# rust-seq/simd-minimizers

Measured on AMD Instinct MI355X. Metric: Gbases/s (whole node) for canonical minimizers k=21 w=11 on 3.1 Gbp; HBM GB/s %peak, higher is better.
Workload: dtype u32

## Files before the change

include/simd_minimizers_amd.h:

```cpp
#ifndef SIMD_MINIMIZERS_AMD_H
#define SIMD_MINIMIZERS_AMD_H

#include <stddef.h>
#include <stdint.h>

#ifdef __cplusplus
extern "C" {
#endif


typedef struct mm_hasher {
    uint32_t fw[4];
    uint32_t rc[4];
    uint32_t rot;
    uint32_t canonical;
    uint32_t fw_xor;
    uint32_t rc_xor;
    uint32_t kind;
} mm_hasher_t;

typedef enum mm_hasher_kind { MM_HASHER_NT = 0, MM_HASHER_MUL = 1, MM_HASHER_ANTILEX = 2 } mm_hasher_kind_t;

typedef enum mm_mode { MM_MINIMIZERS = 0, MM_CLOSED_SYNCMERS = 1, MM_OPEN_SYNCMERS = 2 } mm_mode_t;

// ... 564 lines not shown
int mm_device_group_batch_result(const mm_device_group_t *group, uint64_t seq, int *entry, uint32_t **d_pos,
                                 uint32_t **d_sk, uint64_t *count);
int mm_device_group_gather_batch(mm_device_group_t *group, int root, uint32_t *d_dst_pos, uint32_t *d_dst_sk ,
                                 uint64_t capacity, uint64_t *out_offsets );
int mm_device_group_values_batch(mm_device_group_t *group, uint32_t len, int canonical, int want_u128, uint64_t *total);
int mm_device_group_batch_values(const mm_device_group_t *group, uint64_t seq, int *entry, uint64_t **d_values,
                                 uint64_t *count);

int mm_debug_launch_plan(uint32_t w, int canonical_windows, int mode, uint64_t n_seqs, const uint64_t *n_windows,
                         uint64_t *out7, uint32_t *tile_seq, uint32_t *tile_win0, uint32_t *tile_nblk,
                         uint64_t tile_capacity, uint64_t *n_tiles);
int mm_debug_launch_lds(uint32_t w, int canonical_windows, int mode, uint64_t n_windows, uint64_t *out2);
int mm_debug_fixed_k_kernel(uint32_t k, uint32_t w, int canonical_windows);
int mm_debug_kc_count(uint32_t w, uint32_t k, uint32_t kn, uint32_t jj, uint32_t group, const uint8_t *bytes,
                      uint64_t n_bytes, int64_t lane_base, uint32_t *count);
#define MM_TRAIT_WIDE_GROUP_BLOCKS 0
#define MM_TRAIT_WIDE_DWORDS 1
#define MM_TRAIT_V2_LOAD 2
#define MM_TRAIT_VIEW_WORDS 3
#define MM_TRAIT_AMB_VIEW_WORDS 4
#define MM_TRAIT_SK_SHIFT 5
#define MM_TRAIT_AMBI_LAND 6
#define MM_TRAIT_AMBI_ROWS 7
#define MM_TRAIT_AMB_ROW_DWORDS 8
#define MM_TRAIT_LAZY_VOTE 9
#define MM_TRAIT_TABLE_PREFETCH 10
#define MM_TRAIT_TWO_BODIES 11
#define MM_TRAIT_ENTRY8 12
#define MM_TRAIT_ONE_STREAM 13
#define MM_TRAIT_LAST_VIEW_BASES 14
// ... 17 lines not shown
```

simd-minimizers_amd/__init__.py:

```python
from __future__ import annotations

import ctypes as C
import os
import threading

import numpy as np

_HERE = os.path.dirname(os.path.abspath(__file__))
LIB_PATH = os.environ.get("MM_LIB_PATH") or os.path.join(_HERE, "libsimd_minimizers_amd.so")

MM_MINIMIZERS, MM_CLOSED_SYNCMERS, MM_OPEN_SYNCMERS = 0, 1, 2
PATH_FUSED, PATH_GENERIC, PATH_SPLIT = 1, 2, 3
U64_MAX = (1 << 64) - 1

ERR = {
    "W_ZERO": -1, "W_TOO_LARGE": -2, "LEN_TOO_LARGE": -3, "EVEN_L": -4,
    "HASHER_NOT_CANONICAL": -5, "OPEN_EVEN_W": -6, "K_ZERO": -7, "CAPACITY": -8, "BAD_MODE": -9,
    "NULL": -10, "VALUE_LEN": -11, "FORMAT": -12, "NO_DEVICE": -20, "HIP": -21, "ALLOC": -22, "ORDER": -23,
    "UNSORTED": -24,
}


class MinimizerError(RuntimeError):
    def __init__(self, code: int, msg: str):
# ... 133 lines not shown
                                                           C.c_uint32, vp, vp, C.c_uint64, vp, vp]
            L.mm_run_packed_reads_device.argtypes = [vp, vp, vp, C.c_uint64, C.c_uint64, C.c_uint64, vp, C.c_uint64,
                                                     C.c_uint32, vp, vp, C.c_uint64, vp, u64p]
            L.mm_run_packed_reads_host.argtypes = [vp, vp, u8p, C.c_uint64, u64p, C.c_uint32, u32p, u32p, C.c_uint64, u64p, u64p]
            L.mm_debug_launch_plan.argtypes = [C.c_uint32, C.c_int, C.c_int, C.c_uint64, u64p, u64p, u32p, u32p, u32p,
                                               C.c_uint64, u64p]
        L.mm_clock_probe_begin.argtypes = [vp, C.c_uint64]
        L.mm_clock_probe_end.argtypes = [vp, C.POINTER(C.c_double)]
        L.mm_link_probe.argtypes = [vp, vp, vp, C.c_uint64, C.POINTER(C.c_double)]
        L.mm_debug_launch_lds.argtypes = [C.c_uint32, C.c_int, C.c_int, C.c_uint64, u64p]
        L.mm_debug_fixed_k_kernel.argtypes = [C.c_uint32, C.c_uint32, C.c_int]
        if hasattr(L, "mm_debug_kc_count"):
            L.mm_debug_kc_count.argtypes = [C.c_uint32, C.c_uint32, C.c_uint32, C.c_uint32, C.c_uint32, u8p, C.c_uint64,
                                            C.c_int64, u32p]
            L.mm_debug_kc_count.restype = C.c_int
        if hasattr(L, "mm_debug_walk_traits"):
            L.mm_debug_walk_traits.argtypes = [C.c_uint32, C.c_int, C.c_int, C.c_int, C.c_int, C.c_int, u32p, C.c_int]
            L.mm_debug_walk_traits.restype = C.c_int
        L.mm_debug_lane_plan.argtypes = [C.c_uint32, C.c_uint32, C.c_int, C.c_int, C.c_uint64, C.c_uint64, C.c_uint32, u64p]
        L.mm_debug_last_lane_table.argtypes = [vp, u32p, C.c_uint64, u64p]
        L.mm_fused_overread_bytes.argtypes = []
        L.mm_fused_overread_bytes.restype = C.c_uint64
        L.mm_workspace_force_generic.argtypes = [vp, C.c_int]
        L.mm_workspace_set_blocks_per_lane.argtypes = [vp, C.c_uint32]
        L.mm_workspace_enable_timing.argtypes = [vp, C.c_int]
        L.mm_workspace_kernel_time.argtypes = [vp, C.POINTER(C.c_double), u64p, C.c_int]
        L.mm_workspace_last_path.argtypes = [vp]
        L.mm_workspace_ticket_mode.argtypes = [vp]
        L.mm_workspace_last_lane_table.argtypes = [vp]
        if hasattr(L, "mm_prebuilt_window_sizes"):
# ... 228 lines not shown
    "mm_debug_text_counts_view",
    "mm_run_packed_reads_counts_device_async", "mm_run_packed_reads_counts_device",
    "mm_run_packed_reads_skip_ambiguous_counts_device_async", "mm_run_packed_reads_skip_ambiguous_counts_device",
    "mm_debug_lane_counts_view",
    "mm_fastx_stream_create", "mm_fastx_stream_feed", "mm_fastx_stream_finish", "mm_fastx_stream_next",
    "mm_fastx_stream_destroy", "mm_debug_fastx_cut", "mm_fastx_stream_pieces", "mm_debug_fastx_split",
    "mm_one_minimizer_reads_device_async", "mm_one_minimizer_text_batch_device_async", "mm_one_minimizer_reads_host",
    "mm_one_minimizer_text_batch_host", "mm_one_minimizer_tile", "mm_debug_one_minimizer_reads",
    "mm_debug_one_minimizer_text_batch",
    "mm_one_minimizer_text_batch_counts_device_async", "mm_one_minimizer_reads_counts_device_async",
    "mm_debug_one_minimizer_counts_view", "mm_debug_one_minimizer_text_batch_counts", "mm_debug_one_minimizer_reads_counts",
    "mm_fastx_text_stream_create", "mm_fastx_text_stream_extras",
    "mm_one_minimizer_reads_skip_ambiguous_device_async", "mm_one_minimizer_reads_skip_ambiguous_counts_device_async",
    "mm_one_minimizer_reads_skip_ambiguous_host", "mm_debug_one_minimizer_reads_skip_ambiguous",
    "mm_debug_one_minimizer_reads_skip_ambiguous_counts", "mm_fastx_stream_one_minimizer",
    "mm_debug_walk_traits", "mm_debug_kc_count",
    "mm_bgzf_scan_host", "mm_bgzf_inflate_device_async", "mm_bgzf_inflate_host", "mm_debug_bgzf_inflate",
    "mm_fastx_stream_feed_bgzf",
]

WALK_TRAITS = ("wide_group_blocks", "wide_dwords", "v2_load", "view_words", "amb_view_words", "sk_shift", "ambi_land",
               "ambi_rows", "amb_row_dwords", "lazy_vote", "table_prefetch", "two_bodies", "entry8", "one_stream",
               "last_view_bases")


def walk_traits(w: int, canonical: bool, mode: int = 0, super_kmers: bool = False, reads: bool = False,
                ambiguous: bool = False) -> dict:
    L = lib()
    n = L.mm_debug_walk_traits(int(w), int(canonical), int(mode), int(super_kmers), int(reads), int(ambiguous), None, 0)
    if n != len(WALK_TRAITS):
        raise RuntimeError(f"mm_debug_walk_traits lists {n} values, this package knows {len(WALK_TRAITS)}")
# ... 2125 lines not shown
```

simd-minimizers_amd/csrc/mm_api.hip:

```cpp
#include <hip/hip_runtime.h>

#include <cstdio>
#include <cstdlib>
#include <chrono>
#include <cstring>
#include <new>
#include <algorithm>
#include <string>
#include <thread>
#include <utility>
#include <vector>

#include "../../include/simd_minimizers_amd.h"
#include "mm_env.h"
#include "mm_launch.h"
#include "mm_fasta_text.h"
#include "mm_lane_counts.h"
#include "mm_text_counts.h"
#include "mm_values_batch.h"
#include "mm_values_block.h"
#include "mm_one_min.h"
#include "mm_values_reads.h"
#include "mm_values_text.h"
#include "mm_bgzf.h"
// ... 960 lines not shown
    mm::fused_debug_lds(a, o);
    out2[0] = o[0];
    out2[1] = o[1];
    return MM_OK;
}

int mm_debug_fixed_k_kernel(uint32_t k, uint32_t w, int canonical_windows) {
    return mm::fused_fixed_k(k, w, canonical_windows, canonical_windows) ? 1 : 0;
}

int mm_debug_kc_count(uint32_t w, uint32_t k, uint32_t kn, uint32_t jj, uint32_t group, const uint8_t *bytes, uint64_t n_bytes,
                      int64_t lane_base, uint32_t *count) {
    return mm::fused_kc_count(w, k, kn, jj, group, bytes, n_bytes, lane_base, count);
}

static_assert(MM_WALK_TRAITS == mm::kWalkTraits, "the header's trait indices and fused_walk_traits list the same fields");
int mm_debug_walk_traits(uint32_t w, int canonical_windows, int mode, int super_kmers, int reads, int ambiguous, uint32_t *out,
                         int capacity) {
    if (w == 0 || mode < 0 || mode > 2) return 0;
    return mm::fused_walk_traits(w, canonical_windows != 0, (uint32_t)mode, super_kmers != 0, reads != 0, ambiguous != 0, out,
                                 capacity < 0 ? 0 : capacity);
}

int mm_debug_launch_plan(uint32_t w, int canonical_windows, int mode, uint64_t n_seqs, const uint64_t *n_windows,
                         uint64_t *out7, uint32_t *tile_seq, uint32_t *tile_win0, uint32_t *tile_nblk, uint64_t tile_capacity,
                         uint64_t *n_tiles) {
    ApiScope api_scope;
    if (!n_windows || w == 0) return MM_ERR_NULL;
    mm::RunArgs a = debug_plan_args(w, canonical_windows, mode, n_seqs, n_windows[0]);
    if (n_seqs == 0) {
// ... 4382 lines not shown
```

simd-minimizers_amd/csrc/mm_fused.hip:

```cpp
#include "mm_fused_impl.h"
#include "mm_fused_inst.h"
#include "mm_env.h"
#include "mm_launch.h"
#include "mm_split.h"

#include <cstdlib>
#include <cstdio>
#include <map>
#include <mutex>
#include <string>
#include <utility>
#include <vector>

namespace mm {

namespace {

using KernelFn = FusedKernelFn;
using Instance = FusedInstance;

uint32_t debug_switches() {
#ifdef MM_EXPERIMENTS
    const char *dbg = mm_exp_env("MM_DEBUG");
    return dbg ? (uint32_t)atoi(dbg) : 0u;
// ... 23 lines not shown
    }
    return nullptr;
}

const FusedKcInstance *find_kc_instance(uint32_t w, uint32_t k, int canonical_windows, int hasher_canonical) {
    if (mm_exp_env("MM_NO_KC")) return nullptr;
    int n = 0;
    const FusedKcInstance *inst = fused_kc_instances(&n);
    for (int i = 0; i < n; ++i)
        if (inst[i].w == w && inst[i].k == k && inst[i].canon == (canonical_windows != 0) &&
            inst[i].hash_rc == (hasher_canonical != 0))
            return &inst[i];
    return nullptr;
}

double emit_density(uint32_t w, uint32_t mode) {
    return mode == 2 ? 1.0 / w : (mode == 1 ? 2.0 / w : 2.0 / (w + 1.0));
}

uint32_t list_capacity(uint32_t w, uint32_t mode, uint32_t S) {
    static const uint32_t extra = mm_exp_env("MM_CAP_EXTRA") ? (uint32_t)atoi(mm_exp_env("MM_CAP_EXTRA")) : 0u;
    uint32_t cap = (uint32_t)(1.3 * emit_density(w, mode) * S) + 8u + extra;
    return cap > S + w ? S + w : cap;
}

uint64_t status_stride_host() {
    static const uint64_t v = mm_exp_env("MM_STATUS_STRIDE_HOST") ? (uint64_t)atoi(mm_exp_env("MM_STATUS_STRIDE_HOST")) : kStatusStride;
    return v < kStatusStride ? kStatusStride : v;
}

// ... 20 lines not shown
static uint32_t ambi_landing(uint32_t w, const void *wamb) {
    return wamb ? ambi_land_bytes((int)w) : 0u;
}

struct Geometry {
    uint32_t nblk, S, NB, list_cap, lds_bytes;
    uint64_t nblocks;
};


constexpr uint32_t kMaxLdsBytes = 159u * 1024u;


bool entry8(const RunArgs &a) { return kEntry8Rule(a.w, a.canonical_windows != 0, a.out.sk != nullptr && a.mode == 0); }
uint32_t stride_of(const RunArgs &a) { return list_stride(entry8(a)); }

Geometry geometry(const RunArgs &a) {
    Geometry g;
    g.nblk = legal_nblk(a.w, a.mode, a.nblk, default_cap_limit(a.w, a.canonical_windows != 0, entry8(a)));
    if (entry8(a)) {
        const uint32_t max_nblk = (255u - a.w) / a.w;
        if (g.nblk > max_nblk && !mm_exp_env("MM_E8_NOLIMIT")) g.nblk = max_nblk;
    }
    if (a.nblk == 0 && a.work_windows != 0) {
        const uint64_t fit = a.work_windows / (1024ull * kFusedThreads * a.w);
        if (fit < g.nblk) g.nblk = fit < 6u ? 6u : (uint32_t)fit;
    }
    if (a.nblk == 0 && a.wamb && a.w >= 21u && a.w <= 40u && !ambi_rows_rule((int)a.w)) {
        const uint32_t lim = 400u / a.w;
        if (g.nblk > lim) g.nblk = lim < 6u ? 6u : lim;
    }
    if (a.nblk == 0 && a.wamb && ambi_rows_rule((int)a.w) && a.w <= 54u) {
        const uint32_t per_cu = a.w <= 37u ? 4u : 3u;
        const uint32_t room = (160u * 1024u / per_cu / 1280u) * 1280u - 512u - ambi_land_bytes((int)a.w);
        while (g.nblk > 6u && list_capacity(a.w, a.mode, a.w * g.nblk) * stride_of(a) > room) --g.nblk;
    }
    if (a.out.sk && a.mode == 0) {
        uint32_t sh = 1;
        while ((1u << sh) <= a.w) ++sh;
        while (g.nblk > 1u && ((uint64_t)a.w * g.nblk << sh) > 65536u) --g.nblk;
    }
    for (;;) {
        g.S = a.w * g.nblk;
        const uint32_t cap = list_capacity(a.w, a.mode, g.S);
        g.list_cap = cap;
        g.lds_bytes = cap * stride_of(a);
        if (g.lds_bytes + ambi_landing(a.w, a.wamb) <= kMaxLdsBytes || g.nblk == 1) break;
        g.nblk = g.nblk > 4 ? g.nblk * 7 / 8 : g.nblk - 1;
    }
    g.NB = kFusedThreads * g.S;
// ... 8 lines not shown

struct KernelRef {
    KernelFn host = nullptr;
    hipFunction_t mod = nullptr;
    explicit operator bool() const { return host || mod; }
};

thread_local std::string t_jit_error;

KernelRef resolve_kernel(uint32_t w, int canonical_windows, int hasher_canonical, uint32_t mode, bool sk, uint32_t k = 0,
                         int *how = nullptr) {
    KernelRef kr;
    if (how) *how = kJitHit;
    if (mode > 2) return kr;
    const bool force_jit = force_jit_wanted();
    if (k != 0 && mode == 0 && !sk && !force_jit) {
        if (const FusedKcInstance *kc = find_kc_instance(w, k, canonical_windows, hasher_canonical)) {
            kr.host = kc->fn;
            return kr;
        }
    }
    const Instance *inst = force_jit ? nullptr : find_instance(w, canonical_windows, hasher_canonical);
    if (inst) {
        kr.host = inst->fn[(mode == 0 && sk) ? 3 : mode];
        return kr;
    }
    kr.mod = jit_fused_kernel(w, canonical_windows != 0, hasher_canonical != 0, (int)mode, mode == 0 && sk,
                              false, &t_jit_error, false, how);
    return kr;
}

int launch_kernel(const KernelRef &kr, uint32_t grid, uint32_t lds_bytes, hipStream_t stream, FusedParams &p,
                  hipEvent_t ev0, hipEvent_t ev1) {
    if (kr.host) {
        if (lds_bytes > 64u * 1024u &&
// ... 118 lines not shown
        return b;
    };
    const Buf cur = group_buf(group), prv = group == 0 ? warm_buf() : group_buf(group - 1u);
    const uint32_t s = (gp0 << 1) & 6u;
    uint32_t c = 0;
    for (int i = 0; i < P.n; ++i) {
        const KcCountPiece &pc = P.pc[i];
        const Buf &src = pc.cur ? cur : prv;
        const uint32_t v = alignbit(pc.pair + 1 < ND ? src.q[pc.pair + 1] : 0u, src.q[pc.pair], s + (uint32_t)pc.add);
        c += (uint32_t)__builtin_popcount(v & pc.mask);
    }
    *count = c;
    return rules | 4;
}

static uint32_t whole_rounds_lo(uint32_t nblk) { return nblk * 85u / 100u > 6u ? nblk * 85u / 100u : 6u; }

static uint64_t taper_extra_tiles() {
    int cus = 0, dev = 0;
    if (hipGetDevice(&dev) != hipSuccess ||
        hipDeviceGetAttribute(&cus, hipDeviceAttributeMultiprocessorCount, dev) != hipSuccess || cus < 1) {
        (void)hipGetLastError();
        cus = 512;
    }
    return 8ull * (uint64_t)cus + 64ull;
}

uint64_t fused_status_words(const RunArgs &a) {
    const Geometry g = geometry(a);
    uint64_t tiles = g.nblocks;
// ... 54 lines not shown
    *cus_out = cus;
    return true;
}

template <class TilesFn>
static uint32_t whole_rounds_nblk(const RunArgs &a, const KernelRef &kr, const Geometry &g, TilesFn tiles_of) {
    static const bool off = getenv("MM_NO_ROUNDS") != nullptr;
    if (off || a.nblk != 0 || g.nblocks <= 512) return g.nblk;
    int per_cu = 0, cus = 0;
    const uint32_t land = ambi_landing(a.w, a.wamb);
    if (!resident_slots(kr, g.lds_bytes + land, &per_cu, &cus)) return g.nblk;
    const double slots = 0.98 * per_cu * cus;
    const double kOverheadBlocks = 2.4;
    if ((double)g.nblocks / slots >= 24.0 || (double)g.nblocks / slots <= 1.0) return g.nblk;
    const uint32_t lds_share = (kMaxLdsBytes - (uint32_t)per_cu * 512u) / (uint32_t)per_cu;
    const uint32_t lds_limit = lds_share > land ? lds_share - land : 0u;
    uint32_t sh = 0;
    if (a.out.sk && a.mode == 0)
        for (sh = 1; (1u << sh) <= a.w;) ++sh;
    double best = 0.0;
    uint32_t best_nb = g.nblk;
    const uint32_t lo = whole_rounds_lo(g.nblk), hi = g.nblk * 115u / 100u;
    for (uint32_t nb = lo; nb <= hi; ++nb) {
        const uint64_t S = (uint64_t)a.w * nb;
        if (S > kFusedMaxLaneWindows || (sh && (S << sh) > 65536u)) continue;
        if (list_capacity(a.w, a.mode, (uint32_t)S) * stride_of(a) > lds_limit) continue;
        if (entry8(a) && S + a.w > 255u) continue;
        const double rounds = (double)tiles_of(S) / slots;
        const double cost = (double)(uint64_t)(rounds + 0.999999) * (nb + kOverheadBlocks);
        if (best == 0.0 || cost < best * 0.995 || (nb == g.nblk && cost <= best * 1.005)) {
            best = cost;
// ... 713 lines not shown
```

simd-minimizers_amd/csrc/mm_fused_impl.h:

```cpp
#pragma once
#include "mm_common.h"

#ifndef MM_LB_SLEEP_SHORT
#define MM_LB_SLEEP_SHORT 120
#endif
#ifndef MM_LB_SLEEP_CANON
#define MM_LB_SLEEP_CANON 32
#endif
#ifndef MM_STORE_MOD
#define MM_STORE_MOD "nt"
#endif
#ifndef MM_STORE_AUX
#define MM_STORE_AUX 2
#endif
#ifndef MM_PREFETCH_BLOCKS
#define MM_PREFETCH_BLOCKS 2
#endif
#ifdef MM_STAGE
#define MM_STAGE_GE(n) (MM_STAGE >= (n))
#else
#define MM_STAGE_GE(n) 1
#endif

#ifndef MM_STATUS_STRIDE
// ... 270 lines not shown
    }
    P.ok = t == bits;
    return P;
}
constexpr bool kc_count_rule(int W, int KC) {
#ifdef MM_EAGER_COUNT
    return false;
#endif
    if (!kc_rule(W, KC) || !lazy_vote_rule(W, true)) return false;
    for (int KN = 0; KN < wide_group_blocks(W); ++KN)
        for (int jj = 0; jj < W; ++jj)
            if (!kc_count_plan(W, KC, KN, jj).ok) return false;
    return true;
}

template <int N>
struct IntTag {
    static constexpr int value = N;
};

template <int I, int N, class F>
__device__ __forceinline__ void static_case(const uint32_t i, F &&f) {
    if constexpr (I < N) {
        if (i == (uint32_t)I) f(IntTag<I>{});
        else static_case<I + 1, N>(i, f);
    }
}

template <bool B>
struct BoolTag {
// ... 5 lines not shown
    long long p0;
    uint32_t lane_bases;
    uint32_t wbase;
    bool no_prev;
    int rem_valid;
    int min_rem;
    uint8_t *list;
    uint32_t list_bytes;
    uint32_t list_used;
    unsigned long long dst;
    uint32_t abase;
    uint32_t nblk;
    const uint32_t *seq_d;
    uint32_t seq_dwords;
    uint32_t land;
};

constexpr uint32_t kLandQ4Bytes = 64u * 4u;
constexpr uint32_t amb_row_dwords(int W) { return W <= 37 ? 8u : (W <= 54 ? 11u : 16u); }
#ifndef MM_AMBI_LAND
#define MM_AMBI_LAND 1
#endif
#ifndef MM_AMBI_ROWS_MINW
#define MM_AMBI_ROWS_MINW 36
#endif
constexpr bool ambi_land_rule(int W) { return MM_AMBI_LAND && W >= 32 && W <= 96 && wide_group_blocks(W) != 0; }
constexpr bool ambi_rows_rule(int W) { return ambi_land_rule(W) && W >= MM_AMBI_ROWS_MINW; }
constexpr uint32_t land_amb_bytes(int W) { return ambi_rows_rule(W) ? amb_row_dwords(W) * 256u : 2u * 64u * 16u; }
constexpr uint32_t land_q4_bytes(int W) { return (ambi_rows_rule(W) ? 2u : 4u) * kLandQ4Bytes; }
constexpr uint32_t land_wave_bytes(int W) { return land_amb_bytes(W) + land_q4_bytes(W); }
// ... 66 lines not shown
                const uint2 t = *reinterpret_cast<const uint2 *>(tabb + 128 + a8);
                fw = __builtin_amdgcn_alignbit(fw, fw, rot_l) ^ t.x;
                if (HASH_RC) rc = __builtin_amdgcn_alignbit(rc, rc, rot_r) ^ t.y;
            }
        }
    }

    uint32_t ring_l[W], ring_r[W];
    uint32_t pos_in = pb + k;
    uint32_t pos_out = pb;
    uint32_t kmask;
    asm volatile("v_mov_b32 %0, 0xffff0000" : "=v"(kmask));
    uint32_t m33, m55;
    asm volatile("v_mov_b32 %0, 0x33333333" : "=v"(m33));
    asm volatile("v_mov_b32 %0, 0x55555555" : "=v"(m55));

    uint32_t va[NSUB], vr[NSUB], v2[NSUB];
    constexpr bool kV2Load = v2_load_rule(W, CANON);
    auto next_base_view = [&](const uint32_t (&v)[NSUB], int g) -> uint32_t {
        return g + 1 < NSUB ? __builtin_amdgcn_alignbit(v[g + 1 < NSUB ? g + 1 : g], v[g], 2u) : (v[g] >> 2);
    };
    constexpr int PFD = MM_PREFETCH_BLOCKS;
    RawView qa[PFD - 1][NSUB], qr[PFD - 1][NSUB], q2[PFD - 1][NSUB];
    constexpr int MG = kWideGroup<W>;
    constexpr int ND = kWideDwords<W>;
    struct WideBuf {
        uint32_t q[5];
        uint32_t sh;
    };
#ifdef MM_EXP_ONE_STREAM
// ... 275 lines not shown
#ifndef MM_GROUP_UNROLL
#define MM_GROUP_UNROLL 1
#endif
#ifndef MM_GROUP_UNROLL_PARTIAL
#define MM_GROUP_UNROLL_PARTIAL 1
#endif
    constexpr bool kGroupUnroll = MM_GROUP_UNROLL && MG > 1 && !AMBI && !DIRECT &&
                                  (!PARTIAL || (MM_GROUP_UNROLL_PARTIAL && (kTwoBodies<W> || MM_GROUP_UNROLL_PARTIAL > 1) && MODE == 0 && !SK));
    auto block = [&](const uint32_t b, auto kn_tag) {
        constexpr int KN = decltype(kn_tag)::value;
        uint32_t me[NSUB], mo[NSUB];
        uint32_t tgw[NSUB];
        uint32_t xt[NSUB], yt[NSUB];
#pragma unroll
        for (int g = 0; g < NSUB; ++g) {
#if !defined(MM_VGPR_MASKS) || MM_VGPR_MASKS
            me[g] = select3(m33, va[g], vr[g] << 2);
            mo[g] = select3(m33, va[g] >> 2, vr[g]);
#else
            me[g] = (va[g] & 0x33333333u) | ((vr[g] << 2) & 0xccccccccu);
            mo[g] = ((va[g] >> 2) & 0x33333333u) | (vr[g] & 0xccccccccu);
#endif
            if (CANON) {
                const uint32_t x = va[g], y = v2[g];
                if (!kLazyVote) {
#if !defined(MM_VGPR_MASKS) || MM_VGPR_MASKS
                tgw[g] = select3(m55, (x ^ y) >> 1, y & ~x);
#else
                tgw[g] = (((x ^ y) >> 1) & 0x55555555u) | ((y & ~x) & 0xAAAAAAAAu);
#endif
                } else if (!kCount) {
                const int kCnt = (W - 16 * g) >= 16 ? 16 : (W - 16 * g);
                const uint32_t kBlockMask = 0xAAAAAAAAu & (kCnt >= 16 ? 0xffffffffu : ((1u << (2 * (kCnt > 0 ? kCnt : 0))) - 1u));
                xt[g] = x & kBlockMask;
                yt[g] = y & kBlockMask;
                }
            }
// ... 126 lines not shown
            }
        }
#endif

        const uint32_t e0 = b * (uint32_t)W;
        uint32_t pl = 0, pr_ = 0;
        constexpr int PF = table_prefetch_rule(W, CANON, MG);
        uint2 tq[W];
        auto lookup = [&](int j) -> uint2 {
            const int jj = j & 15, g = j >> 4, m = jj >> 1;
            const uint32_t mw = (jj & 1) ? mo[g] : me[g];
            const uint32_t a8 = (m == 0 ? (mw << 3) : (mw >> (4 * m - 3))) & 0x78u;
            if (!MM_STAGE_GE(2)) return uint2{a8, a8};
            return *reinterpret_cast<const uint2 *>(tabb + a8);
        };
#pragma unroll
        for (int j = 0; j < PF; ++j) tq[j] = lookup(j);
        auto steps = [&](auto fe_tag) {
        constexpr int FEK = (int)decltype(fe_tag)::value;
        constexpr bool FE = FEK != 0;
        auto emit_step = [&](const int jj, uint32_t sel, const unsigned long long valid) {
            const uint32_t e = e0 + (uint32_t)jj;
            const uint32_t i = e - (uint32_t)W;
            if (FE) {
                unsigned long long sv;
                if (FEK == 2) {
                    uint32_t selx, st;
                    const uint32_t m = (uint32_t)__builtin_amdgcn_sbfe((int)aw[AMBI ? (jj >> 5) : 0], jj & 31, 1);
                    asm("v_or_b32 %0, %1, %2" : "=v"(selx) : "v"(sel), "v"(m));
                    asm("v_bitop3_b32 %0, %1, %2, %2 bitop3:0x30" : "=v"(st) : "v"(stride_v), "v"(m));
#define MM_EMIT_SKIP(WR, SELB)                                                                        \
    asm volatile("v_cmp_ne_u32_sdwa vcc, %[sel], %[prev] src0_sel:" SELB " src1_sel:" SELB "\n\t"    \
// ... 170 lines not shown
                    });
                });
                return c <= (uint32_t)thr ? selr : sel;
            }
            int d = dn;
#pragma unroll
            for (int g = 0; g <= (jj >> 4); ++g) {
                const int nb = jj - 16 * g;
                const uint32_t m = nb >= 16 ? 0xAAAAAAAAu : (0xAAAAAAAAu & ((1u << (2 * (nb > 0 ? nb : 0))) - 1u));
                if (m) d += (int)__builtin_popcount(xt[g] & m) - (int)__builtin_popcount(yt[g] & m);
            }
            return d < 0 ? selr : sel;
        };
        uint32_t p_sel = 0, p_selr = 0;
        unsigned long long p_differ = 0ull, p_valid = ~0ull;
#pragma unroll
        for (int j = 0; j < W; ++j) {
            const uint32_t e = e0 + (uint32_t)j;
            if (j + PF < W) tq[j + PF] = lookup(j + PF);
            const uint32_t h = HASH_RC ? fw + rc : fw;
#ifdef MM_STAGE
            if (!MM_STAGE_GE(3)) {
                const uint2 t0 = tq[j];
                if (MM_STAGE_GE(2)) {
                    fw = __builtin_amdgcn_alignbit(fw, fw, rot_l) ^ t0.x;
                    if (HASH_RC) rc = __builtin_amdgcn_alignbit(rc, rc, rot_r) ^ t0.y;
                    sink ^= h;
                } else {
                    sink += t0.x;
                }
                continue;
            }
#endif
            const uint32_t kl = and_or3(h, kmask, e);
// ... 31 lines not shown
                    }
                }
            }
#ifdef MM_STAGE
            if (!MM_STAGE_GE(5)) {
                sink ^= sel;
                const uint2 t0 = tq[j];
                fw = __builtin_amdgcn_alignbit(fw, fw, rot_l) ^ t0.x;
                if (HASH_RC) rc = __builtin_amdgcn_alignbit(rc, rc, rot_r) ^ t0.y;
                if (CANON && !kLazyVote && MM_STAGE_GE(4)) dn += __builtin_amdgcn_sbfe((int)tgw[j >> 4], 2 * (j & 15), 2);
                continue;
            }
#endif
            if (!deferred) emit_step(j, sel, valid);

            const uint2 t = tq[j];
            fw = __builtin_amdgcn_alignbit(fw, fw, rot_l) ^ t.x;
            if (HASH_RC) rc = __builtin_amdgcn_alignbit(rc, rc, rot_r) ^ t.y;
            if (CANON && !kLazyVote) dn += __builtin_amdgcn_sbfe((int)tgw[j >> 4], 2 * (j & 15), 2);
        }
        if (CANON && kLazyVote && MM_STAGE_GE(5) && !(MM_VOTE_NO_DEFER)) {
            if (__builtin_expect(p_differ != 0ull, 0)) p_sel = decide(W - 1, p_sel, p_selr, p_differ);
            emit_step(W - 1, p_sel, p_valid);
        }
        };
        constexpr bool kCanFast = !DIRECT;
        if (kCanFast && !PARTIAL && !AMBI) {
            steps(IntTag<1>{});
        } else if (kRangeFE) {
            steps(IntTag<kRangeFE ? 1 : 0>{});
        } else if (kCanFast && kTwoBodies<W>) {
            bool ok = true;
            if (AMBI) {
// ... 364 lines not shown
#define MM_MIN_BLOCKS_WALK MM_MIN_BLOCKS
#endif
__global__ __launch_bounds__(kFusedThreads, MM_MIN_BLOCKS) void fused_kernel(const FusedParams p) {
    extern __shared__ __attribute__((aligned(16))) uint8_t smem[];
    __shared__ uint2 s_tab[36];
    __shared__ uint32_t s_bid;
    __shared__ uint32_t s_overflow;
    __shared__ uint32_t s_done;
    __shared__ uint32_t s_wave_tot[kFusedWaves];
    __shared__ unsigned long long s_excl;

    constexpr bool kAmbi = CANON && !SK;
    constexpr bool kE8 = kEntry8<W, CANON, SK, READS>;
    constexpr uint32_t kStride = list_stride(kE8), kEB = kE8 ? 1u : 2u;
    const int tid = threadIdx.x, lane = tid & (kWave - 1), wave = tid / kWave;
    {
        auto lds_end = [](const void *q, size_t bytes) {
            return (uint32_t)reinterpret_cast<uintptr_t>(q) + (uint32_t)bytes;
        };
        uint32_t st_end = lds_end(s_tab, sizeof(s_tab));
        st_end = max(st_end, lds_end(&s_bid, sizeof(s_bid)));
        st_end = max(st_end, lds_end(&s_overflow, sizeof(s_overflow)));
        st_end = max(st_end, lds_end(&s_done, sizeof(s_done)));
        st_end = max(st_end, lds_end(s_wave_tot, sizeof(s_wave_tot)));
        st_end = max(st_end, lds_end(&s_excl, sizeof(s_excl)));
        if ((uint32_t)reinterpret_cast<uintptr_t>(smem) < st_end) {
            if (tid == 0) flag_error(p.out.error, 2u);
            return;
        }
    }
    const bool redo = !READS && p.redo_list != nullptr;
    if (redo && blockIdx.x >= *p.redo_n) return;
    if (tid == 0) {
        s_bid = redo ? p.redo_list[blockIdx.x].tile : (p.use_ticket ? atomicAdd(p.out.ticket, 1u) : blockIdx.x);
        s_overflow = redo ? 1u : 0u;
        s_done = 0;
    }
    if (tid < 16) s_tab[tid] = p.ht.t_in_out[tid];
    else if (tid < 20) s_tab[tid] = p.ht.t_in[tid - 16];
    else if (tid < 36) s_tab[tid] = p.ht.t_in2[tid - 20];
    __syncthreads();
    const uint32_t bid = __builtin_amdgcn_readfirstlane(s_bid);
    const unsigned long long etag = (unsigned long long)p.epoch << kEpochShift;
    if ((MM_DBG(p) & 32u) && bid == 0 && tid == 0) flag_error(p.out.error, 1u);
    if (p.trace && tid == 0) {
        uint32_t hw, xcc;
        asm volatile("s_getreg_b32 %0, hwreg(HW_REG_HW_ID)" : "=s"(hw));
        asm volatile("s_getreg_b32 %0, hwreg(HW_REG_XCC_ID)" : "=s"(xcc));
        p.trace[10 * (size_t)bid + 0] = wall_clock64();
        p.trace[10 * (size_t)bid + 4] = ((unsigned long long)xcc << 32) | hw;
    }

    uint32_t nblk_t = p.nblk;
    unsigned long long tile_off = 0;
    bool tapered = false;
// ... 45 lines not shown
        p.trace[10 * (size_t)bid + 6] = (unsigned long long)reinterpret_cast<uintptr_t>(seq_d);
        p.trace[10 * (size_t)bid + 7] = ((unsigned long long)seq_dwords << 32) | seq_base0;
        p.trace[10 * (size_t)bid + 8] = ((unsigned long long)win_end << 32) | local_tile;
        p.trace[10 * (size_t)bid + 9] = batch_s;
    }
    const uint64_t bw0 = READS ? 0ull
                     : batch ? (uint64_t)batch_win0
                             : (uint64_t)win_begin + (tapered ? tile_off : (uint64_t)local_tile * NB);
    const uint32_t nvalid = READS ? NB
        : (uint32_t)(((uint64_t)win_end - bw0) < NB ? ((uint64_t)win_end - bw0) : NB);
    const bool partial = READS || nvalid < NB;

    uint8_t *const lists = smem + p.land_bytes;
    LaneCtx ctx;
    ctx.tab = s_tab;
    ctx.list = lists + kEB * (uint32_t)tid;
    ctx.list_bytes = p.list_cap * kStride;
    ctx.dst = 0;
    ctx.nblk = nblk_t;
    ctx.seq_d = seq_d;
    ctx.seq_dwords = seq_dwords;
    ctx.land = 0;
    if (kAmbi && ambi_land_rule(W) && p.wamb) {
        if (p.land_bytes < ambi_land_bytes(W)) {
            if (tid == 0) flag_error(p.out.error, 4u);
            return;
        }
        ctx.land = __builtin_amdgcn_readfirstlane((uint32_t)reinterpret_cast<uintptr_t>(smem) + (uint32_t)wave * land_wave_bytes(W));
    }
    bool lane_active = false;
// ... 331 lines not shown
```

simd-minimizers_amd/csrc/mm_launch.h:

```cpp
#pragma once
#include <hip/hip_runtime.h>
#include <stdint.h>

#include <initializer_list>
#include <string>
#include <vector>

#include "mm_common.h"
#include "mm_values_reads.h"

namespace mm {

struct RunArgs {
    SeqView seq;
    HashTables ht;
    uint32_t k, w;
    int canonical_windows;
    uint32_t mode;
    uint64_t win_begin, win_end;
    OutParams out;
    const uint32_t *wamb;
    uint32_t wamb_dwords;
    const BatchSeq *batch_seqs;
    const BatchTile *batch_tile_seq;
// ... 15 lines not shown
uint64_t fused_overread_bytes();

bool fused_supported(uint32_t k, uint32_t w, int canonical_windows, int hasher_canonical);
bool fused_fixed_k(uint32_t k, uint32_t w, int canonical_windows, int hasher_canonical);
uint64_t fused_status_words(const RunArgs &a);
uint64_t fused_status_stride();
uint32_t fused_tile_windows(const RunArgs &a);
uint32_t fused_batch_nblk(const RunArgs &a, const uint64_t *n_windows, uint64_t n_seqs);
int fused_debug_plan(const RunArgs &a, unsigned long long *out );
void fused_debug_lds(const RunArgs &a, unsigned long long *out2);
constexpr int kWalkTraits = 15;
int fused_walk_traits(uint32_t w, bool canonical_windows, uint32_t mode, bool sk, bool reads, bool ambiguous, uint32_t *out,
                      int capacity);
int fused_kc_count(uint32_t w, uint32_t k, uint32_t kn, uint32_t jj, uint32_t group, const uint8_t *bytes, uint64_t n_bytes,
                   int64_t lane_base, uint32_t *count);
bool fused_batch_tiles(const RunArgs &a, const uint64_t *n_windows, uint64_t n_seqs, std::vector<BatchTile> &tiles,
                       uint32_t *nblk_out);
int launch_fused(const RunArgs &a, hipStream_t stream);
const char *fused_unavailable_reason();
int fused_prebuilt_windows(bool canonical, bool reads, uint32_t *out, int capacity);
int fused_prebuilt_flavour_windows(bool canonical, bool reads, uint32_t mode, bool sk, uint32_t *out, int capacity);

struct PrepareCounts {
    uint32_t kernels = 0, compiled = 0, from_disk = 0, unavailable = 0;
};
inline hipError_t load_kernels(std::initializer_list<const void *> fns, uint32_t *kernels) {
    for (const void *fn : fns) {
        hipFuncAttributes fa{};
        const hipError_t e = hipFuncGetAttributes(&fa, fn);
        if (e != hipSuccess) {
// ... 191 lines not shown
```

Before: 2151.

## Use paired-base hash lookup table to advance rolling hash two steps per load

Adds a 256-entry LDS table, built per workgroup, that covers each pair of consecutive in/out base pairs. It holds the single-step xor terms and the combined two-step terms for the forward and reverse-complement rolling hashes. For canonical minimizers with odd w and a fixed-k kernel, the window loop now does one 16-byte lookup every two steps instead of one 8-byte lookup per step, using a 4-bit nibble mask in place of the 2-bit one. It also shrinks the block count when needed to leave room for the extra 4 KB of static LDS. This trades fewer LDS lookups for extra LDS use, which may lower occupancy or tile size, plus some added register pressure from the wider prefetched entries.

```diff
diff --git a/include/simd_minimizers_amd.h b/include/simd_minimizers_amd.h
--- a/include/simd_minimizers_amd.h
+++ b/include/simd_minimizers_amd.h
@@ -602,6 +602,7 @@
 int mm_debug_fixed_k_kernel(uint32_t k, uint32_t w, int canonical_windows);
 int mm_debug_kc_count(uint32_t w, uint32_t k, uint32_t kn, uint32_t jj, uint32_t group, const uint8_t *bytes,
                       uint64_t n_bytes, int64_t lane_base, uint32_t *count);
+int mm_debug_pair_table(const mm_hasher_t *h, uint32_t out[1024]);
 #define MM_TRAIT_WIDE_GROUP_BLOCKS 0
 #define MM_TRAIT_WIDE_DWORDS 1
 #define MM_TRAIT_V2_LOAD 2
diff --git a/simd-minimizers_amd/__init__.py b/simd-minimizers_amd/__init__.py
--- a/simd-minimizers_amd/__init__.py
+++ b/simd-minimizers_amd/__init__.py
@@ -171,6 +171,9 @@
             L.mm_debug_kc_count.argtypes = [C.c_uint32, C.c_uint32, C.c_uint32, C.c_uint32, C.c_uint32, u8p, C.c_uint64,
                                             C.c_int64, u32p]
             L.mm_debug_kc_count.restype = C.c_int
+        if hasattr(L, "mm_debug_pair_table"):
+            L.mm_debug_pair_table.argtypes = [C.POINTER(Hasher), u32p]
+            L.mm_debug_pair_table.restype = C.c_int
         if hasattr(L, "mm_debug_walk_traits"):
             L.mm_debug_walk_traits.argtypes = [C.c_uint32, C.c_int, C.c_int, C.c_int, C.c_int, C.c_int, u32p, C.c_int]
             L.mm_debug_walk_traits.restype = C.c_int
@@ -429,7 +432,7 @@
     "mm_one_minimizer_reads_skip_ambiguous_device_async", "mm_one_minimizer_reads_skip_ambiguous_counts_device_async",
     "mm_one_minimizer_reads_skip_ambiguous_host", "mm_debug_one_minimizer_reads_skip_ambiguous",
     "mm_debug_one_minimizer_reads_skip_ambiguous_counts", "mm_fastx_stream_one_minimizer",
-    "mm_debug_walk_traits", "mm_debug_kc_count",
+    "mm_debug_walk_traits", "mm_debug_kc_count", "mm_debug_pair_table",
     "mm_bgzf_scan_host", "mm_bgzf_inflate_device_async", "mm_bgzf_inflate_host", "mm_debug_bgzf_inflate",
     "mm_fastx_stream_feed_bgzf",
 ]
diff --git a/simd-minimizers_amd/csrc/mm_api.hip b/simd-minimizers_amd/csrc/mm_api.hip
--- a/simd-minimizers_amd/csrc/mm_api.hip
+++ b/simd-minimizers_amd/csrc/mm_api.hip
@@ -998,6 +998,12 @@
     return mm::fused_kc_count(w, k, kn, jj, group, bytes, n_bytes, lane_base, count);
 }
 
+int mm_debug_pair_table(const mm_hasher_t *h, uint32_t out[1024]) {
+    if (!h || !out) return MM_ERR_NULL;
+    mm::fused_pair_table(make_tables(*h, 21), out);
+    return MM_OK;
+}
+
 static_assert(MM_WALK_TRAITS == mm::kWalkTraits, "the header's trait indices and fused_walk_traits list the same fields");
 int mm_debug_walk_traits(uint32_t w, int canonical_windows, int mode, int super_kmers, int reads, int ambiguous, uint32_t *out,
                          int capacity) {
diff --git a/simd-minimizers_amd/csrc/mm_fused.hip b/simd-minimizers_amd/csrc/mm_fused.hip
--- a/simd-minimizers_amd/csrc/mm_fused.hip
+++ b/simd-minimizers_amd/csrc/mm_fused.hip
@@ -61,6 +61,17 @@
     return nullptr;
 }
 
+const FusedKcInstance *launch_kc_instance(uint32_t w, int canonical_windows, int hasher_canonical, uint32_t mode, bool sk,
+                                          uint32_t k) {
+    if (k == 0 || mode != 0 || sk || force_jit_wanted()) return nullptr;
+    return find_kc_instance(w, k, canonical_windows, hasher_canonical);
+}
+
+uint32_t extra_static_lds(uint32_t w, int canonical_windows, int hasher_canonical, uint32_t mode, bool sk, uint32_t k) {
+    if (!launch_kc_instance(w, canonical_windows, hasher_canonical, mode, sk, k)) return 0u;
+    return pair_lookup_rule((int)w, canonical_windows != 0, (int)k, (int)mode, sk, false, false) ? kPairTableBytes : 0u;
+}
+
 double emit_density(uint32_t w, uint32_t mode) {
     return mode == 2 ? 1.0 / w : (mode == 1 ? 2.0 / w : 2.0 / (w + 1.0));
 }
@@ -111,6 +122,10 @@
 
 bool entry8(const RunArgs &a) { return kEntry8Rule(a.w, a.canonical_windows != 0, a.out.sk != nullptr && a.mode == 0); }
 uint32_t stride_of(const RunArgs &a) { return list_stride(entry8(a)); }
+uint32_t extra_static_lds_of(const RunArgs &a) {
+    return extra_static_lds(a.w, a.canonical_windows, (int)a.ht.canonical, a.mode, a.out.sk != nullptr, a.k);
+}
+constexpr uint32_t kPairWorkgroupLds = 160u * 1024u / 4u;
 
 Geometry geometry(const RunArgs &a) {
     Geometry g;
@@ -131,6 +146,12 @@
         const uint32_t per_cu = a.w <= 37u ? 4u : 3u;
         const uint32_t room = (160u * 1024u / per_cu / 1280u) * 1280u - 512u - ambi_land_bytes((int)a.w);
         while (g.nblk > 6u && list_capacity(a.w, a.mode, a.w * g.nblk) * stride_of(a) > room) --g.nblk;
+    }
+    if (a.nblk == 0) {
+        if (const uint32_t st = extra_static_lds_of(a)) {
+            const uint32_t room = kPairWorkgroupLds - 512u - st - ambi_landing(a.w, a.wamb);
+            while (g.nblk > 6u && list_capacity(a.w, a.mode, a.w * g.nblk) * stride_of(a) > room) --g.nblk;
+        }
     }
     if (a.out.sk && a.mode == 0) {
         uint32_t sh = 1;
@@ -169,11 +190,9 @@
     if (how) *how = kJitHit;
     if (mode > 2) return kr;
     const bool force_jit = force_jit_wanted();
-    if (k != 0 && mode == 0 && !sk && !force_jit) {
-        if (const FusedKcInstance *kc = find_kc_instance(w, k, canonical_windows, hasher_canonical)) {
-            kr.host = kc->fn;
-            return kr;
-        }
+    if (const FusedKcInstance *kc = launch_kc_instance(w, canonical_windows, hasher_canonical, mode, sk, k)) {
+        kr.host = kc->fn;
+        return kr;
     }
     const Instance *inst = force_jit ? nullptr : find_instance(w, canonical_windows, hasher_canonical);
     if (inst) {
@@ -322,6 +341,16 @@
     return rules | 4;
 }
 
+void fused_pair_table(const HashTables &ht, uint32_t *out1024) {
+    for (uint32_t i = 0; i < kPairEntries; ++i) {
+        const uint4 e = pair_entry(ht, i);
+        out1024[4 * i + 0] = e.x;
+        out1024[4 * i + 1] = e.y;
+        out1024[4 * i + 2] = e.z;
+        out1024[4 * i + 3] = e.w;
+    }
+}
+
 static uint32_t whole_rounds_lo(uint32_t nblk) { return nblk * 85u / 100u > 6u ? nblk * 85u / 100u : 6u; }
 
 static uint64_t taper_extra_tiles() {
@@ -406,7 +435,8 @@
     const double kOverheadBlocks = 2.4;
     if ((double)g.nblocks / slots >= 24.0 || (double)g.nblocks / slots <= 1.0) return g.nblk;
     const uint32_t lds_share = (kMaxLdsBytes - (uint32_t)per_cu * 512u) / (uint32_t)per_cu;
-    const uint32_t lds_limit = lds_share > land ? lds_share - land : 0u;
+    const uint32_t beside = land + extra_static_lds_of(a);
+    const uint32_t lds_limit = lds_share > beside ? lds_share - beside : 0u;
     uint32_t sh = 0;
     if (a.out.sk && a.mode == 0)
         for (sh = 1; (1u << sh) <= a.w;) ++sh;
diff --git a/simd-minimizers_amd/csrc/mm_fused_impl.h b/simd-minimizers_amd/csrc/mm_fused_impl.h
--- a/simd-minimizers_amd/csrc/mm_fused_impl.h
+++ b/simd-minimizers_amd/csrc/mm_fused_impl.h
@@ -308,6 +308,26 @@
     return true;
 }
 
+constexpr bool pair_lookup_rule(int W, bool CANON, int KC, int MODE, bool SK, bool READS, bool AMBI) {
+#ifdef MM_NO_PAIR
+    return false;
+#endif
+    return CANON && MODE == 0 && !SK && !READS && !AMBI && (W & 1) == 1 && kc_rule(W, KC);
+}
+constexpr uint32_t kPairEntries = 256u;
+constexpr uint32_t kPairTableBytes = kPairEntries * 16u;
+__host__ __device__ inline uint4 pair_entry(const HashTables &ht, const uint32_t idx) {
+    const uint32_t in4 = idx & 15u, out4 = (idx >> 4) & 15u;
+    const uint2 t1 = ht.t_in_out[((out4 & 3u) << 2) | (in4 & 3u)], t2 = ht.t_in_out[(out4 & 12u) | (in4 >> 2)];
+    const uint32_t r = ht.rot & 31u;
+    uint4 e;
+    e.x = t1.x;
+    e.y = t1.y;
+    e.z = (r ? (t1.x << r) | (t1.x >> (32u - r)) : t1.x) ^ t2.x;
+    e.w = (r ? (t1.y >> r) | (t1.y << (32u - r)) : t1.y) ^ t2.y;
+    return e;
+}
+
 template <int N>
 struct IntTag {
     static constexpr int value = N;
@@ -343,6 +363,7 @@
     const uint32_t *seq_d;
     uint32_t seq_dwords;
     uint32_t land;
+    const uint4 *pair;
 };
 
 constexpr uint32_t kLandQ4Bytes = 64u * 4u;
@@ -439,6 +460,9 @@
     uint32_t m33, m55;
     asm volatile("v_mov_b32 %0, 0x33333333" : "=v"(m33));
     asm volatile("v_mov_b32 %0, 0x55555555" : "=v"(m55));
+    constexpr bool kPair = pair_lookup_rule(W, CANON, KC, MODE, SK, false, AMBI);
+    uint32_t m0f = 0;
+    if constexpr (kPair) asm volatile("v_mov_b32 %0, 0x0f0f0f0f" : "=v"(m0f));
 
     uint32_t va[NSUB], vr[NSUB], v2[NSUB];
     constexpr bool kV2Load = v2_load_rule(W, CANON);
@@ -744,6 +768,10 @@
         uint32_t xt[NSUB], yt[NSUB];
 #pragma unroll
         for (int g = 0; g < NSUB; ++g) {
+            if constexpr (kPair) {
+                me[g] = select3(m0f, va[g], vr[g] << 4);
+                mo[g] = select3(m0f, va[g] >> 4, vr[g]);
+            } else {
 #if !defined(MM_VGPR_MASKS) || MM_VGPR_MASKS
             me[g] = select3(m33, va[g], vr[g] << 2);
             mo[g] = select3(m33, va[g] >> 2, vr[g]);
@@ -751,6 +779,7 @@
             me[g] = (va[g] & 0x33333333u) | ((vr[g] << 2) & 0xccccccccu);
             mo[g] = ((va[g] >> 2) & 0x33333333u) | (vr[g] & 0xccccccccu);
 #endif
+            }
             if (CANON) {
                 const uint32_t x = va[g], y = v2[g];
                 if (!kLazyVote) {
@@ -907,8 +936,24 @@
             if (!MM_STAGE_GE(2)) return uint2{a8, a8};
             return *reinterpret_cast<const uint2 *>(tabb + a8);
         };
+        static_assert(!kPair || (PF % 2 == 0 && PF >= 2 && PF <= W), "pair look-ups are issued at even steps");
+        uint4 tqp[(W + 1) / 2];
+        auto lookup_pair = [&](int q) -> uint4 {
+            const int g = q >> 3, qq = q & 7, byte = qq >> 1;
+            const uint32_t mw = (qq & 1) ? mo[g] : me[g];
+            const uint32_t a16 = ((mw >> (8 * byte)) & 0xffu) << 4;
+            const uint8_t *pairb = reinterpret_cast<const uint8_t *>(ctx.pair);
+            if (2 * q + 1 < W) return *reinterpret_cast<const uint4 *>(pairb + a16);
+            const uint2 t1 = *reinterpret_cast<const uint2 *>(pairb + a16);
+            return uint4{t1.x, t1.y, 0u, 0u};
+        };
+        if constexpr (kPair) {
+#pragma unroll
+            for (int q = 0; 2 * q < PF; ++q) tqp[q] = lookup_pair(q);
+        } else {
 #pragma unroll
         for (int j = 0; j < PF; ++j) tq[j] = lookup(j);
+        }
         auto steps = [&](auto fe_tag) {
         constexpr int FEK = (int)decltype(fe_tag)::value;
         constexpr bool FE = FEK != 0;
@@ -1109,10 +1154,15 @@
         };
         uint32_t p_sel = 0, p_selr = 0;
         unsigned long long p_differ = 0ull, p_valid = ~0ull;
+        uint32_t fwk = fw, rck = rc;
 #pragma unroll
         for (int j = 0; j < W; ++j) {
             const uint32_t e = e0 + (uint32_t)j;
+            if constexpr (kPair) {
+                if (((j + PF) & 1) == 0 && j + PF < W) tqp[(j + PF) >> 1] = lookup_pair((j + PF) >> 1);
+            } else {
             if (j + PF < W) tq[j + PF] = lookup(j + PF);
+            }
             const uint32_t h = HASH_RC ? fw + rc : fw;
 #ifdef MM_STAGE
             if (!MM_STAGE_GE(3)) {
@@ -1174,9 +1224,22 @@
 #endif
             if (!deferred) emit_step(j, sel, valid);
 
+            if constexpr (kPair) {
+                const uint4 t = tqp[j >> 1];
+                if ((j & 1) == 0) {
+                    fwk = fw;
+                    rck = rc;
+                    fw = __builtin_amdgcn_alignbit(fwk, fwk, rot_l) ^ t.x;
+                    if (HASH_RC) rc = __builtin_amdgcn_alignbit(rck, rck, rot_r) ^ t.y;
+                } else {
+                    fw = __builtin_amdgcn_alignbit(fwk, fwk, rot2_l) ^ t.z;
+                    if (HASH_RC) rc = __builtin_amdgcn_alignbit(rck, rck, rot2_r) ^ t.w;
+                }
+            } else {
             const uint2 t = tq[j];
             fw = __builtin_amdgcn_alignbit(fw, fw, rot_l) ^ t.x;
             if (HASH_RC) rc = __builtin_amdgcn_alignbit(rc, rc, rot_r) ^ t.y;
+            }
             if (CANON && !kLazyVote) dn += __builtin_amdgcn_sbfe((int)tgw[j >> 4], 2 * (j & 15), 2);
         }
         if (CANON && kLazyVote && MM_STAGE_GE(5) && !(MM_VOTE_NO_DEFER)) {
@@ -1571,6 +1634,15 @@
     constexpr bool kE8 = kEntry8<W, CANON, SK, READS>;
     constexpr uint32_t kStride = list_stride(kE8), kEB = kE8 ? 1u : 2u;
     const int tid = threadIdx.x, lane = tid & (kWave - 1), wave = tid / kWave;
+    constexpr bool kPair = pair_lookup_rule(W, CANON, KC, MODE, SK, READS, false);
+    uint4 *pair_tab = nullptr;
+    uint32_t pair_end = 0;
+    if constexpr (kPair) {
+        static_assert(kFusedThreads == kPairEntries, "one pair-table entry per thread");
+        __shared__ uint4 s_pair[kPairEntries];
+        pair_tab = s_pair;
+        pair_end = (uint32_t)reinterpret_cast<uintptr_t>(s_pair) + (uint32_t)sizeof(s_pair);
+    }
     {
         auto lds_end = [](const void *q, size_t bytes) {
             return (uint32_t)reinterpret_cast<uintptr_t>(q) + (uint32_t)bytes;
@@ -1581,6 +1653,7 @@
         st_end = max(st_end, lds_end(&s_done, sizeof(s_done)));
         st_end = max(st_end, lds_end(s_wave_tot, sizeof(s_wave_tot)));
         st_end = max(st_end, lds_end(&s_excl, sizeof(s_excl)));
+        if constexpr (kPair) st_end = max(st_end, pair_end);
         if ((uint32_t)reinterpret_cast<uintptr_t>(smem) < st_end) {
             if (tid == 0) flag_error(p.out.error, 2u);
             return;
@@ -1596,6 +1669,7 @@
     if (tid < 16) s_tab[tid] = p.ht.t_in_out[tid];
     else if (tid < 20) s_tab[tid] = p.ht.t_in[tid - 16];
     else if (tid < 36) s_tab[tid] = p.ht.t_in2[tid - 20];
+    if constexpr (kPair) pair_tab[tid] = pair_entry(p.ht, (uint32_t)tid);
     __syncthreads();
     const uint32_t bid = __builtin_amdgcn_readfirstlane(s_bid);
     const unsigned long long etag = (unsigned long long)p.epoch << kEpochShift;
@@ -1671,6 +1745,7 @@
     uint8_t *const lists = smem + p.land_bytes;
     LaneCtx ctx;
     ctx.tab = s_tab;
+    if constexpr (kPair) ctx.pair = pair_tab;
     ctx.list = lists + kEB * (uint32_t)tid;
     ctx.list_bytes = p.list_cap * kStride;
     ctx.dst = 0;
diff --git a/simd-minimizers_amd/csrc/mm_launch.h b/simd-minimizers_amd/csrc/mm_launch.h
--- a/simd-minimizers_amd/csrc/mm_launch.h
+++ b/simd-minimizers_amd/csrc/mm_launch.h
@@ -53,6 +53,7 @@
                       int capacity);
 int fused_kc_count(uint32_t w, uint32_t k, uint32_t kn, uint32_t jj, uint32_t group, const uint8_t *bytes, uint64_t n_bytes,
                    int64_t lane_base, uint32_t *count);
+void fused_pair_table(const HashTables &ht, uint32_t *out1024);
 bool fused_batch_tiles(const RunArgs &a, const uint64_t *n_windows, uint64_t n_seqs, std::vector<BatchTile> &tiles,
                        uint32_t *nblk_out);
 int launch_fused(const RunArgs &a, hipStream_t stream);
```

Result: faster. 2178, median of 6 (+1.3%).
